# datasciencetoolkit/NextGP.jl

Measured on AMD Instinct MI355X. Metric: gibbs_iterations_per_sec, higher is better.
Workload: dtype f64; 1 GPU; single-trait Gibbs sweep, N=50000 individuals x P=600000 SNPs, marker sets BayesPR(200000) + BayesPR(200000) + BayesPR(200000), fp32 panel in HBM (BASELINE.json configs[3]: multi-breed random regression = three BayesPR marker sets of 200,000 SNPs); N=50000, P=600000, chains=1, panel_dtype=f32, accumulate_dtype=f64

## Files before the change

__graft_entry__.py:

```python
import os
import subprocess
import sys

ROOT = os.path.dirname(os.path.abspath(__file__))
PKG = os.path.join(ROOT, "nextgp.jl_amd")
CSRC = os.path.join(PKG, "csrc")
LIB = os.path.join(PKG, "libnextgp_hip.so")
HIPCC = os.environ.get("HIPCC", "/opt/rocm/bin/hipcc")
HIP_FLAGS = ["--offload-arch=gfx950", "-O3", "-std=c++17", "-ffp-contract=off", "-fPIC"]
OBJ_DIR = os.path.join(ROOT, "build", "obj")
_SWEEP_DEPS = ["ngp_sweep_inst.hip", "ngp_sweep.h", "ngp_sweep_body.inc", "ngp_sweep_multi_body.inc", "ngp_sweep_args.h", "ngp_common.h", "ngp_rng.h"]
UNITS = [("ngp_api.o", "ngp_api.hip", [], ["ngp_api.hip", "ngp_kernels.h", "ngp_state.h", "ngp_random.h", "ngp_random_tuple.h", "ngp_dense.h", "ngp_logvar.h", "ngp_bayesrc.h", "ngp_predict.h", "ngp_holdout.h", "ngp_genvar.h", "ngp_sweep_args.h", "ngp_common.h", "ngp_rng.h"]),
         ("ngp_genvar.o", "ngp_genvar_inst.hip", [], ["ngp_genvar_inst.hip", "ngp_genvar.h", "ngp_common.h"]),
         ("ngp_sweep_0.o", "ngp_sweep_inst.hip", ["-DNGP_INST_DBG=0"], _SWEEP_DEPS),
         ("ngp_sweep_1.o", "ngp_sweep_inst.hip", ["-DNGP_INST_DBG=1"], _SWEEP_DEPS),
         ("ngp_sweep_2.o", "ngp_sweep_inst.hip", ["-DNGP_INST_DBG=2"], _SWEEP_DEPS),
         ("ngp_sweep_3.o", "ngp_sweep_inst.hip", ["-DNGP_INST_DBG=3"], _SWEEP_DEPS),
         ("ngp_sweep_4.o", "ngp_sweep_inst.hip", ["-DNGP_INST_DBG=4"], _SWEEP_DEPS)]


def _stale(target, sources):
    if not os.path.exists(target):
        return True
    t = os.path.getmtime(target)
    return any(os.path.getmtime(s) > t for s in sources)


def build(force=False):
    srcs = [os.path.join(CSRC, f) for f in sorted(os.listdir(CSRC))] + [os.path.join(ROOT, "include", "nextgp_hip.h")]
    if force or _stale(LIB, srcs):
        os.makedirs(OBJ_DIR, exist_ok=True)
        procs = []
        hdr = os.path.join(ROOT, "include", "nextgp_hip.h")
# ... 57 lines not shown
```

nextgp.jl_amd/_lib.py:

```python
import ctypes as C
import os

import numpy as np

_HERE = os.path.dirname(os.path.abspath(__file__))
LIB_PATH = os.environ.get("NGP_HIP_LIB") or os.path.join(_HERE, "libnextgp_hip.so")

METHOD_BAYESPR, METHOD_BAYESB, METHOD_BAYESC, METHOD_BAYESR, METHOD_TUPLE, METHOD_BAYESLV, METHOD_BAYESRC = 0, 1, 2, 3, 4, 5, 6
LV_MAXCOV, LV_WORDS = 16, 17


def _sample_header(f, path):
    magic = f.read(8)
    if magic not in (b"NGPSMP01", b"NGPSMP02", b"NGPSMP03", b"NGPSMP04"):
        raise NextGPHipError(f"not a sample file: {path}")
    P, nvb, nsets, nfix, ncls, rec = (int(v) for v in np.frombuffer(f.read(48), dtype=np.int64))
    sets = [dict(zip(("method", "K", "col0", "ncol", "nvb", "tk"), np.frombuffer(f.read(48), dtype=np.int64).tolist())) for _ in range(nsets)]
    rq = []
    if magic in (b"NGPSMP02", b"NGPSMP03", b"NGPSMP04"):
        nr = int(np.frombuffer(f.read(8), dtype=np.int64)[0])
        rq = np.frombuffer(f.read(8 * nr), dtype=np.int64).tolist()
    lv = []
    if magic in (b"NGPSMP03", b"NGPSMP04"):
        nl = int(np.frombuffer(f.read(8), dtype=np.int64)[0])
# ... 955 lines not shown
    def set_trace_loci(self, loci, n_varBeta=0):
        loci = np.ascontiguousarray(loci, dtype=np.int64)
        self._chk(self.L.ngp_set_trace_loci(self.h, _p(loci, C.c_int64) if len(loci) else None, C.c_int64(len(loci)), C.c_int64(n_varBeta)))
        self.ntl, self.ntvb = len(loci), n_varBeta

    def get_trace_ext(self, n):
        bt = np.empty((n, max(self.ntl, 1))); vt = np.empty((n, max(self.ntvb, 1))); pt = np.empty((n, max(self.nsets, 1)))
        self._chk(self.L.ngp_get_trace_ext(self.h, _p(bt, C.c_double), _p(vt, C.c_double), _p(pt, C.c_double), C.c_int64(n)))
        return dict(beta=bt[:, :self.ntl], varBeta=vt[:, :self.ntvb], pi=pt[:, :self.nsets])

    def census(self):
        g, r, e = C.c_int64(), C.c_int64(), C.c_int32()
        self._chk(self.L.ngp_get_census(self.h, None, C.c_int64(0), C.byref(g), C.byref(r), C.byref(e)))
        tb = np.zeros(g.value, dtype=np.uint64)
        self._chk(self.L.ngp_get_census(self.h, _p(tb, C.c_uint64), C.c_int64(g.value), None, None, None))
        return dict(grid=g.value, retries=r.value, exclusive=bool(e.value), xcc=(tb >> np.uint64(32)).astype(np.int64) - 1,
                    hw_id=(tb & np.uint64(0xFFFFFFFF)).astype(np.int64))

    def warmer(self):
        a, b = C.c_int32(), C.c_int64()
        self._chk(self.L.ngp_get_warmer(self.h, C.byref(a), C.byref(b)))
        return dict(active=a.value, blocks=b.value)

    def debug_fail_census(self, iteration):
        self._chk(self.L.ngp_debug_fail_census(self.h, C.c_int64(iteration)))

    def debug_set_virtual_device(self, vdev):
        self._chk(self.L.ngp_debug_set_virtual_device(self.h, C.c_int32(vdev)))

    @staticmethod
    def allreduce_posterior(samplers):
        L = samplers[0].L
# ... 30 lines not shown
```

nextgp.jl_amd/csrc/ngp_api.hip:

```cpp
#include <hip/hip_runtime.h>
#include <cassert>

#include <dlfcn.h>

#include <algorithm>
#include <chrono>
#include <cmath>
#include <cstdio>
#include <cstdlib>
#include <condition_variable>
#include <cstddef>
#include <cstring>
#include <array>
#include <atomic>
#include <deque>
#include <map>
#include <memory>
#include <mutex>
#include <queue>
#include <string>
#include <thread>
#include <vector>

#include "../../include/nextgp_hip.h"
// ... 199 lines not shown
constexpr size_t NGP_LDS_MAX = 160 * 1024;

void choose_layout(int64_t N, int64_t max_shards, int64_t r_cap, int64_t *R, int64_t *S, bool prefer_odd = true) {
    int64_t r0 = (N + max_shards - 1) / max_shards;
    int64_t m = (r0 + 3) / 4;
    if (m < 1) m = 1;
    if (prefer_odd && (m & 1) == 0 && 4 * (m + 1) <= r_cap) m += 1;
    int64_t r = 4 * m;
    if (r > r_cap) r = r_cap;
    *R = r;
    *S = (N + r - 1) / r;
}

size_t sampler_lds(SweepKernel k) {
    const size_t base = (size_t)(3 * 4096 + 2 * NGP_RING * NGP_BLK + 6 * NGP_BLK) * sizeof(double) + 2 * NGP_BLK * sizeof(int) + 320;
    if (k == SweepKernel::lean) return base;
    if (k == SweepKernel::r || k == SweepKernel::multi_r) return base + NGP_SAMPLER_TUPLE_LDS + NGP_SAMPLER_R_LDS;
    return base + NGP_SAMPLER_TUPLE_LDS;
}

size_t streamer_lds(const SweepPlan &p, int K) {
    const int R = (int)p.R;
    if (K > 1) return p.streamer == 3 ? ngp_rows_multi_lds_bytes(R, K, true) : (p.streamer == 2 ? ngp_rows_multi_lds_bytes(R, K) : ngp_multi_lds_bytes(R, K));
    if (p.streamer >= 2) {
        const size_t nq = (p.streamer == 3) ? (size_t)R / 16 : (size_t)R / 4, hq = std::min<size_t>(NGP_ROWS_HMAX, (nq + 1) / 2);
        return (2 * nq + hq) * NGP_QS + (size_t)p.V * ((R + 7) & ~7) * 8 + 2 * NGP_ROWS_NW * NGP_BLK * 8 + 2 * NGP_DLS * 8 + 16 * 8 + 64 + 1024;
    }
    return 2 * (size_t)(R / 4) * NGP_QS + (size_t)R * 16 + 4096 + 2 * 512 + 128 + 3072 + (size_t)R * 64;
}

size_t sweep_lds(const SweepPlan &p, SweepKernel k, int K = 1) {
// ... 12 lines not shown
        assert(!diag && (K == 1 || p.V == 1));
        return K > 1 ? SweepKernel::multi_rc : (p.V > 1 ? SweepKernel::tall_rc : SweepKernel::rc);
    }
    if (K > 1) {
        if (rset && sweep_lds(p, SweepKernel::multi_r, K) <= NGP_LDS_MAX) return SweepKernel::multi_r;
        return tup ? SweepKernel::multi_tup : SweepKernel::multi;
    }
    if (p.V > 1) return SweepKernel::tall;
    if (diag) return SweepKernel::diag;
    if (rset && sweep_lds(p, SweepKernel::r) <= NGP_LDS_MAX) return SweepKernel::r;
    if (tup || rset) return SweepKernel::tup;
    return SweepKernel::lean;
}

const void *sweep_kernel(SweepKernel k) {
    for (auto unit : {sweep_kernel_0, sweep_kernel_1, sweep_kernel_2, sweep_kernel_3, sweep_kernel_4})
        if (const void *f = unit(k)) return f;
    return nullptr;
}

void launch_sweep_kernel(SweepKernel k, int64_t grid, size_t lds, hipStream_t stream, void *args) {
    void *a[] = {args};
    (void)hipLaunchKernel(sweep_kernel(k), dim3((unsigned)grid), dim3(NGP_WG), a, lds, stream);
}

int plan_sweep(int64_t N, int cu_count, const PlanRequest &q, SweepPlan *out, const char **msg) {
    SweepPlan p;
    p.mode = q.mode;
    int64_t max_shards = cu_count - 1 - (cu_count + NGP_GRP - 1) / NGP_GRP;
    if (q.max_shards_req > 0) max_shards = std::min<int64_t>(max_shards, q.max_shards_req);
    if (q.storage == 1) {
// ... 349 lines not shown
    if ((rc = c.d_ycorr.alloc(h, (size_t)L))) return rc;
    if (!h->h_rw.empty()) {
        std::vector<double> rs((size_t)L, 0.0);
        for (int64_t i = 0; i < N; i++) rs[(size_t)i] = std::sqrt(h->h_rw[(size_t)i]);
        if ((rc = c.d_rs.alloc(h, (size_t)L))) return rc;
        HCHK(hipMemcpy(c.d_rs, rs.data(), rs.size() * sizeof(double), hipMemcpyHostToDevice));
    }
    if ((rc = c.d_part.alloc(h, (size_t)plan.S * NGP_BLK))) return rc;
    if ((rc = c.d_dlt.alloc(h, NGP_BLK))) return rc;
    if ((rc = c.d_sets.alloc(h, 16))) return rc;
    if ((rc = c.d_scal.alloc(h, 1))) return rc;
    HCHK(hipMemsetAsync(c.d_setof, 0xFF, pp, h->stream));
    HCHK(hipMemsetAsync(c.d_delta, 1, pp, h->stream));
    if (req.storage == 0) HCHK(hipFuncSetAttribute((const void *)k_step, hipFuncAttributeMaxDynamicSharedMemorySize, (int)lds_step));
    if (plan.mode == 1) {
        for (SweepKernel k : {SweepKernel::lean, SweepKernel::diag, SweepKernel::tup, SweepKernel::r, SweepKernel::rc, SweepKernel::tall, SweepKernel::tall_rc}) {
            const size_t lds = sweep_lds(plan, k);
            if (lds <= NGP_LDS_MAX) HCHK(hipFuncSetAttribute(sweep_kernel(k), hipFuncAttributeMaxDynamicSharedMemorySize, (int)lds));
        }
        int wg_per_cu = 0;
        const SweepKernel occ = plan.V > 1 ? SweepKernel::tall : SweepKernel::lean;
        HCHK(hipOccupancyMaxActiveBlocksPerMultiprocessor(&wg_per_cu, sweep_kernel(occ), NGP_WG, sweep_lds(plan, SweepKernel::tup)));
        const int64_t grid = sweep_grid(plan);
        if (wg_per_cu < 1 || grid > (int64_t)wg_per_cu * h->cu_count)
            return fail(h, NGP_ERR_STATE, "persistent sweep: grid of " + std::to_string(grid) + " workgroups cannot be co-resident (" +
                                              std::to_string(wg_per_cu) + " per CU x " + std::to_string(h->cu_count) + " CUs); use ngp_configure(mode 0)");
        if ((rc = c.d_cdlt.alloc(h, (size_t)NGP_RING * NGP_BLK))) return rc;
        if ((rc = c.d_cdltg.alloc(h, (size_t)NGP_RING * NGP_BLK * 2))) return rc;
        c.census_off = (size_t)NGP_RING * NGP_FX_COPIES * NGP_BLK * 2 + 32;
        c.ccnt_words = c.census_off + 32 + 2 * (size_t)320;
        if ((rc = c.d_ccnt.alloc(h, c.ccnt_words))) return rc;
// ... 219 lines not shown
        if ((rc = h->mm.d_tseg_len.alloc(h, h->h_tseg_len.size()))) return rc;
        if ((rc = h->mm.d_tseg_set.alloc(h, h->h_tseg_set.size()))) return rc;
        if ((rc = h->mm.d_tsegpart.alloc(h, h->h_tseg_l0.size() * NGP_TPAIRS))) return rc;
        HCHK(hipMemcpy(h->mm.d_tregs, h->h_tregs.data(), h->h_tregs.size() * sizeof(DTReg), hipMemcpyHostToDevice));
        HCHK(hipMemcpy(h->mm.d_tseg_l0, h->h_tseg_l0.data(), h->h_tseg_l0.size() * sizeof(long long), hipMemcpyHostToDevice));
        HCHK(hipMemcpy(h->mm.d_tseg_len, h->h_tseg_len.data(), h->h_tseg_len.size() * sizeof(int32_t), hipMemcpyHostToDevice));
        HCHK(hipMemcpy(h->mm.d_tseg_set, h->h_tseg_set.data(), h->h_tseg_set.size() * sizeof(int32_t), hipMemcpyHostToDevice));
    }
    h->tables_dirty = false;
    return NGP_OK;
}

bool is_kept(const ngp_handle *h, int64_t it) {
    if (it < h->burnIn + h->thin || it > h->chainLength) return false;
    return ((it - h->burnIn) % h->thin) == 0;
}

void fill_sweep_args(ngp_handle *h, int64_t tb0, int64_t tb1, SweepArgs &A) {
    const int R = (int)h->plan.R, S = (int)h->plan.S;
    A.tiles = h->pm->tiles; A.ycorr = h->cm.d_ycorr; A.gramx = h->pm->gramx;
    const bool tf = wants_tinv(h) && h->cm.tinv_blocks == h->NBLK;
    A.tinv = (tf && h->cm.lin_any) ? h->cm.d_tinv : nullptr;
    A.blin = (tf && h->cm.lin_any) ? h->cm.d_blin : nullptr;
    A.lin_all = (tf && h->cm.lin_any) ? h->cm.lin_all : 0;
    A.V = h->plan.V; A.D = h->plan.D; A.R = R; A.S = S; A.NG = h->plan.NG; A.near = h->plan.near; A.fine_ok = 0; A.t0 = (int)tb0; A.t1 = (int)tb1;
    A.beta = h->cm.d_beta; A.delta = h->cm.d_delta; A.c = h->cm.d_c; A.w = h->cm.d_w; A.q = h->cm.d_q; A.mpm = h->pm->mpm; A.chi = h->cm.d_chi;
    A.setof = h->cm.d_setof; A.vbidx = h->cm.d_vbidx; A.sets = h->cm.d_sets; A.varBeta = h->mm.d_varBeta;
    A.rcls = h->mm.d_rcls; A.rhs0 = h->cm.d_rhs0; A.scal = h->cm.d_scal; A.Ppad = h->Ppad;
    A.tup = h->ntuple ? h->mm.d_tup : nullptr; A.tupc = h->mm.d_tupc; A.tupg = h->mm.d_tupg;
    A.acc = (unsigned long long *)h->cm.d_ccnt.get(); A.dlt = h->cm.d_cdlt; A.dltg = h->cm.d_cdltg;
    h->launch_seq = (h->launch_seq % 4095u) + 1u;
    A.nonce = h->launch_seq;
    A.flag_dlt = h->cm.d_ccnt + (size_t)NGP_RING * NGP_FX_COPIES * NGP_BLK * 2; A.abort_w = h->cm.d_abort; A.xcc_w = h->cm.d_abort + 16;
    A.census = (h->dbg_mode == 0) ? h->cm.d_ccnt + h->cm.census_off : nullptr;
    A.census_tbl = h->cm.d_census_tbl; A.iter_tag = (unsigned)(h->iter + 1);
    A.census_fail = (h->dbg_census_fail_iter > 0 && !h->exclusive) ? (unsigned)h->dbg_census_fail_iter : 0u;
    A.dbg = h->hm.d_dbg;
    A.fine_ok = (streamer_lds(h->plan, 1) + 8192 <= sweep_lds(h->plan, SweepKernel::diag)) ? 1 : 0;
    const bool warmer_tall = h->plan.R >= NGP_WARMER_MIN_R || (h->knob & NGP_KNOB_WARMER_ANY_R);
    const bool warmer_idle = h->plan.NG > 0 && h->plan.NG % 8 == 0 && h->plan.near + h->plan.NG >= h->plan.D;
    const bool warmer = h->dbg_mode == 0 && h->plan.streamer == 2 && h->plan.V == 1 && !(h->knob & NGP_KNOB_NO_WARMER) &&
                        warmer_tall && warmer_idle;
    A.variant = h->plan.streamer; A.knob = (h->knob & ~NGP_KNOB_WARMER) | (warmer ? NGP_KNOB_WARMER : 0);
    A.mean = h->pm->mean; A.N = h->N;
    A.dbg_mode = h->dbg_mode;
}

void launch_sweep(ngp_handle *h, int64_t tb0, int64_t tb1, hipEvent_t *evs) {
    const int R = (int)h->plan.R, S = (int)h->plan.S;
    if (h->plan.mode == 1) {
        SweepArgs A;
        fill_sweep_args(h, tb0, tb1, A);
        const SweepKernel k = pick_kernel(h->plan, 1, h->hm.d_dbg || h->dbg_mode, h->ntuple > 0, h->nclass_total > 0, !h->mm.rc.empty());
        h->last_grid = sweep_grid(h->plan);
        if (evs) (void)hipEventRecord(evs[0], h->stream);
        launch_sweep_kernel(k, h->last_grid, sweep_lds(h->plan, k), h->stream, &A);
        if (evs) (void)hipEventRecord(evs[1], h->stream);
        h->sweep_launches += 1;
        return;
    }
    int e = 0;
    for (int64_t t = tb0; t <= tb1; t++) {
        const int do_upd = t > tb0, do_gemv = t < tb1;
        if (evs && do_gemv) (void)hipEventRecord(evs[e++], h->stream);
        hipLaunchKernelGGL(k_step, dim3((unsigned)S), dim3(256), h->lds_step, h->stream, h->pm->tiles, h->cm.d_ycorr, h->cm.d_dlt, h->cm.d_part, R,
                           S, (int)t, do_upd, do_gemv);
        if (evs && do_gemv) (void)hipEventRecord(evs[e++], h->stream);
        if (do_gemv)
// ... 4273 lines not shown
```

nextgp.jl_amd/csrc/ngp_sweep.h:

```cpp
#pragma once
#include <cstddef>
#include <type_traits>
#include "ngp_sweep_args.h"

#ifndef NGP_ROWS_DPP
#define NGP_ROWS_DPP 1
#endif

#pragma clang fp contract(off)

namespace ngp {


#define NGP_DBG_FOLD                                                     \
    unsigned long long *const dbg = DBG ? A.dbg : nullptr;               \
    const int dbg_mode = DBG ? A.dbg_mode : 0;                           \
    (void)dbg; (void)dbg_mode;
#define NGP_DBG_LOCALS                                                   \
    unsigned long long *const dbg = A.dbg;                               \
    const int dbg_mode = A.dbg_mode;                                     \
    (void)dbg; (void)dbg_mode;
#define NGP_DBG_ROWS NGP_DBG_FOLD

__device__ inline unsigned ld_u32(const unsigned *p) { return __hip_atomic_load(p, __ATOMIC_RELAXED, __HIP_MEMORY_SCOPE_AGENT); }
// ... 503 lines not shown
#define NGP_VMC8(b) NGP_VMC(b) NGP_VMC(b + 1) NGP_VMC(b + 2) NGP_VMC(b + 3) NGP_VMC(b + 4) NGP_VMC(b + 5) NGP_VMC(b + 6) NGP_VMC(b + 7)
    switch (n) {
        NGP_VMC(1) NGP_VMC(2) NGP_VMC(3) NGP_VMC(4) NGP_VMC(5) NGP_VMC(6) NGP_VMC(7) NGP_VMC(8) NGP_VMC(9) NGP_VMC(10) NGP_VMC(11)
        NGP_VMC(12) NGP_VMC(13) NGP_VMC(14) NGP_VMC(15) NGP_VMC(16) NGP_VMC(17) NGP_VMC(18) NGP_VMC(19) NGP_VMC(20) NGP_VMC(21)
        NGP_VMC(22) NGP_VMC(23) NGP_VMC(24) NGP_VMC(25) NGP_VMC(26) NGP_VMC(27) NGP_VMC(28) NGP_VMC(29) NGP_VMC(30) NGP_VMC(31)
        NGP_VMC(32) NGP_VMC(33) NGP_VMC(34) NGP_VMC(35) NGP_VMC(36) NGP_VMC(37) NGP_VMC(38) NGP_VMC(39) NGP_VMC(40) NGP_VMC(41)
        NGP_VMC(42) NGP_VMC(43) NGP_VMC(44) NGP_VMC(45) NGP_VMC(46) NGP_VMC(47) NGP_VMC(48) NGP_VMC(49) NGP_VMC(50) NGP_VMC(51)
        NGP_VMC(52) NGP_VMC(53) NGP_VMC(54) NGP_VMC(55) NGP_VMC(56) NGP_VMC(57) NGP_VMC(58) NGP_VMC(59) NGP_VMC(60) NGP_VMC(61)
        NGP_VMC(62) NGP_VMC(63)
        default: asm volatile("s_waitcnt vmcnt(0)" ::: "memory"); break;
    }
#undef NGP_VMC8
#undef NGP_VMC
}

template <bool DBG, int DT, int ST>
__device__ __attribute__((always_inline)) inline void role_streamer_rows(const SweepArgs &A, const int s, char *smem) {
    NGP_DBG_ROWS
    constexpr bool U8 = (ST != 0);
    constexpr int NT = U8 ? ST : 1;
    const int R = A.R, S = A.S, tid = threadIdx.x;
    const int wv = __builtin_amdgcn_readfirstlane(tid >> 6), lane = tid & 63;
    const int NQ = U8 ? (R >> 4) : (R >> 2);
    const int H = min(NGP_ROWS_HMAX, (NQ + 1) >> 1);
    const int RQ = 2 * NQ + H;
    char *ring = smem;
    double *ys = (double *)(smem + (size_t)RQ * NGP_QS);
    double *red = ys + ((R + 7) & ~7);
    double *dl = red + 2 * NGP_ROWS_NW * NGP_BLK;
    double *rsy = dl + 2 * NGP_DLS;
    int *sflag = (int *)(rsy + 16);
    char *scratch = (char *)(rsy + 16) + 64;
    unsigned long long *fine = (unsigned long long *)(scratch + 1024);
    const bool fine_on = DBG && dbg && s == (DBG ? fine_shard(A) : 1) && A.fine_ok == 1;
#define NGP_FINE(k)                                                                                              \
    do {                                                                                                         \
        if (fine_on && (unsigned)(u - 800) < 16u && lane == 0) fine[(((u - 800) * 8 + wv) << 3) + (k)] = wall_clock64(); \
    } while (0)
    const size_t tile_bytes = (size_t)NQ * 1024;
    double *yg = A.ycorr + (size_t)s * R;
    const int g = s / NGP_GRP;
    const int nb = A.t1 - A.t0;
    for (int i = tid; i < R; i += NGP_WG) ys[i] = yg[i];
    int *gcnt0 = (int *)(rsy + 7), *gcnt1 = (int *)(rsy + 15);
    const bool early = U8 ? ((A.knob & 256) != 0) : ((A.knob & 256) == 0);
    if (tid == 0) { *sflag = 1; *gcnt0 = 0; *gcnt1 = 0; }
    int base = 0;
    auto wrap = [&](int p) __attribute__((always_inline)) { return p >= RQ ? p - RQ : p; };
    if (wv == NGP_ROWS_NW) {
        const unsigned ring0 = (unsigned)(size_t)(__attribute__((address_space(3))) const char *)ring;
        const unsigned scratch0 = (unsigned)(size_t)(__attribute__((address_space(3))) const char *)scratch;
        const unsigned voff = (unsigned)lane * 16u;
        const bool no_dma = DBG && dbg_mode == 4;
        const int pace = A.knob & 7;
        auto dma_quads = [&](int tile, int q0, int q1, int tbase) __attribute__((always_inline)) {
            if (no_dma || q0 >= q1) return 0;
            const char *g = (const char *)A.tiles + ((size_t)(A.t0 + tile) * S + s) * tile_bytes + (size_t)q0 * 1024;
            int p = wrap(tbase + q0);
            int q = q0;
            for (; q + 4 <= q1; q += 4) {
                if (p + 4 <= RQ) {
                    dma16_s4(ring0 + (unsigned)p * NGP_QS, g, voff);
// ... 16 lines not shown
            }
            for (; q < q1; ++q) {
                dma16_s(ring0 + (unsigned)p * NGP_QS, g, voff);
                g += 1024;
                if (++p == RQ) p = 0;
            }
            return q1 - q0;
        };
        const unsigned my_xcc = xcc_id() + 1u;
        const int nslice = max(1, S / 8);
        const int slice = (s / 8) % nslice;
        const size_t gram_bytes = warm_bytes(A, min(DT, A.near + 1)), w_thi = warm_t_hi(A), w_shift = warm_shift(A);
        const size_t slice_bytes = ((gram_bytes / nslice + 1023) / 1024) * 1024;
        bool same_xcd = false, xcc_known = false;
        __builtin_amdgcn_s_setprio(3);
        if (nb > 0) dma_quads(0, 0, NQ, 0);
        if (nb > 1) dma_quads(1, 0, H, NQ);
        drain_vm();
        wg_barrier();
        for (int u = 0; u < nb + DT; ++u) {
            NGP_FINE(0);
            const int base1 = wrap(base + NQ), base2 = wrap(base1 + NQ);
            if (!xcc_known && (u & 7) == 0) {
                if constexpr (U8) {
                    const unsigned x = sld_u32(A.xcc_w);
                    xcc_known = (x != 0u);
                    same_xcd = (x == my_xcc);
                } else {
                    unsigned x, wx = 0u;
                    if (A.knob & NGP_KNOB_WARMER) sld_u32x2_glc(A.xcc_w, warmer_words(A), x, wx);
                    else x = sld_u32(A.xcc_w);
                    xcc_known = (x != 0u) && (x != my_xcc || !(A.knob & NGP_KNOB_WARMER) || wx != 0u);
                    same_xcd = (x == my_xcc) && (wx != x) && !(A.knob & NGP_KNOB_NO_WARM);
                }
            }
            if (same_xcd && u + 1 < nb && !no_dma) {
                const char *gb = (const char *)(A.gramx + (size_t)(A.t0 + u + 1) * DT * NGP_BLK * NGP_BLK) - w_shift;
                const char *tb = (const char *)(A.tinv + (size_t)(A.t0 + u + 1) * NGP_BLK * NGP_BLK);
                const size_t lo = (size_t)slice * slice_bytes, hi = min((size_t)(slice + 1) * slice_bytes, gram_bytes);
                for (size_t off = lo; off + 1024 <= hi; off += 1024) dma16_warm(scratch0, (off < w_thi ? tb : gb) + off, voff);
            }
            if (u + 1 < nb) dma_quads(u + 1, H, NQ, base1);
            int n2 = 0;
            if (u + 2 < nb) n2 = dma_quads(u + 2, 0, H, base2);
            NGP_FINE(1);
            wait_vmcnt_le(n2);
            NGP_FINE(2);
            wg_barrier();
            if (!*sflag) return;
            base = base1;
        }
        drain_vm();
    } else {
        const int c = lane & 7, ql = lane >> 3;
        const int nqw = (NQ - wv + NGP_ROWS_NW - 1) / NGP_ROWS_NW;
        int tslot[NT], trow[NT];
        bool thas[NT];
#pragma unroll
        for (int i = 0; i < NT; i++) {
            if constexpr (U8) {
                const int tau = ql + 8 * i;
                thas[i] = (tau >> 2) < nqw;
                tslot[i] = thas[i] ? wv + NGP_ROWS_NW * (tau >> 2) : wv;
                trow[i] = 16 * tslot[i] + 4 * (tau & 3);
            } else {
                const int qt = wv + NGP_ROWS_NW * ql;
                thas[i] = qt < NQ;
                tslot[i] = thas[i] ? qt : wv;
                trow[i] = 4 * qt;
            }
// ... 7 lines not shown
            for (int jj = 0; jj < 8; jj++) {
                if constexpr (U8) {
#pragma unroll
                    for (int i = 0; i < NT; i++) keep8[d][i][jj] = 0u;
                } else {
                    keep[d][jj] = make_float4(0.f, 0.f, 0.f, 0.f);
                }
            }
        unsigned long long pg0 = 0, pg1 = 0;
        double pm = 0.0;
        int pm_blk = -1;
        double mpub = 0.0;
        if (U8 && wv == NGP_ROWS_PUBW && nb > 0) mpub = A.mean[(size_t)A.t0 * NGP_BLK + lane];
        const double fxs = A.scal->fx_scale;
        auto try_signal = [&](bool) __attribute__((always_inline)) {};
        auto publish = [&](const int u) __attribute__((always_inline)) {
            const int slot = u % NGP_RING;
            const double *rp = red + (u & 1) * NGP_ROWS_NW * NGP_BLK + lane;
            double p = ((rp[0] + rp[NGP_BLK]) + (rp[2 * NGP_BLK] + rp[3 * NGP_BLK])) + ((rp[4 * NGP_BLK] + rp[5 * NGP_BLK]) + rp[6 * NGP_BLK]);
            if constexpr (U8) {
                const double *sp = rsy + (u & 1) * 8;
                const double sy = ((sp[0] + sp[1]) + (sp[2] + sp[3])) + ((sp[4] + sp[5]) + sp[6]);
                const double ms = mpub * sy;
                p = p - ms;
            }
            if (U8 && u + 1 < nb) mpub = A.mean[(size_t)(A.t0 + u + 1) * NGP_BLK + lane];
            acc_add(A.acc, A.abort_w, slot, s, lane, p, fxs);
            if (DBG && dbg && s == 0 && lane == 0) dbg[NGP_DBG_STREAM + 2 * (size_t)u] = wall_clock64();
        };
        wg_barrier();
// ... 77 lines not shown
                            }
                            const double q4 = (y0 + y1) + (y2 + y3);
                            vsum = (i == 0) ? q4 : vsum + q4;
                        }
                    }
                    if (u < nb) {
                        vsum = vsum + dpp_f64(vsum, 4);
                        const double r0 = readlane_d(vsum, 0), r1 = readlane_d(vsum, 16), r2 = readlane_d(vsum, 32), r3 = readlane_d(vsum, 48);
                        if (lane == 0) rsy[(u & 1) * 8 + wv] = (r0 + r1) + (r2 + r3);
                    }
                }
                NGP_FINE(1);
                try_signal(false);
                if (u < nb) {
                    double acc = 0.0;
                    for (int k = 0; k < nqw; k++) {
                        const int q = wv + NGP_ROWS_NW * k;
                        if constexpr (U8) {
                            const uint4 x = *(const uint4 *)(ring + (size_t)wrap(base + q) * NGP_QS + (size_t)lane * 16);
                            const double *yq = ys + 16 * q;
                            const unsigned xw[4] = {x.x, x.y, x.z, x.w};
#pragma unroll
                            for (int e4 = 0; e4 < 4; e4++) {
                                const unsigned w = xw[e4];
                                const double y0 = yq[4 * e4], y1 = yq[4 * e4 + 1], y2 = yq[4 * e4 + 2], y3 = yq[4 * e4 + 3];
                                acc = __builtin_fma((double)(float)(w & 0xffu), y0, acc);
                                acc = __builtin_fma((double)(float)((w >> 8) & 0xffu), y1, acc);
                                acc = __builtin_fma((double)(float)((w >> 16) & 0xffu), y2, acc);
                                acc = __builtin_fma((double)(float)(w >> 24), y3, acc);
                            }
                        } else {
// ... 1 lines not shown
#if NGP_ROWS_DPP
                            const double xd[4] = {(double)x.x, (double)x.y, (double)x.z, (double)x.w};
                            double yv[1] = {ys[4 * q + (lane & 3)]}, ac[1] = {acc};
                            fmac4_bcast<1>(ac, yv, xd);
                            acc = ac[0];
#else
                            const double *yq = ys + 4 * q;
                            const double y0 = yq[0], y1 = yq[1], y2 = yq[2], y3 = yq[3];
                            acc = __builtin_fma((double)x.x, y0, acc);
                            acc = __builtin_fma((double)x.y, y1, acc);
                            acc = __builtin_fma((double)x.z, y2, acc);
                            acc = __builtin_fma((double)x.w, y3, acc);
#endif
                        }
                    }
                    red[((u & 1) * NGP_ROWS_NW + wv) * NGP_BLK + lane] = acc;
                    if (early) {
                        asm volatile("" ::: "memory");
                        if (lane == 0) __hip_atomic_fetch_add((lds_int_t *)((u & 1) ? gcnt1 : gcnt0), 1, __ATOMIC_RELAXED, __HIP_MEMORY_SCOPE_WORKGROUP);
                    }
                    NGP_FINE(2);
                    try_signal(false);
                    if constexpr (U8) {
#pragma unroll
                        for (int i = 0; i < NT; i++) {
                            const char *tq = ring + (size_t)wrap(base + tslot[i]) * NGP_QS + c * 128 + (trow[i] & 15);
#pragma unroll
                            for (int jj = 0; jj < 8; jj++) keep8[d][i][jj] = *(const unsigned *)(tq + jj * 16);
                        }
                    } else {
                        const char *tq = ring + (size_t)wrap(base + tslot[0]) * NGP_QS + c * 128;
#pragma unroll
                        for (int jj = 0; jj < 8; jj++) keep[d][jj] = *(const float4 *)(tq + jj * 16);
                    }
                }
                NGP_FINE(3);
                if (early && wv == NGP_ROWS_PUBW && u < nb && !(DBG && dbg_mode == 1)) {
// ... 42 lines not shown
                NGP_FINE(5);
                if (!early && wv == NGP_ROWS_PUBW && u < nb && !(DBG && dbg_mode == 1)) publish(u);
                base = wrap(base + NQ);
                NGP_FINE(6);
            }
        }
        try_signal(true);
    }
    if (fine_on && nb > 816) {
        __syncthreads();
        for (int i = tid; i < 1024; i += NGP_WG) dbg[NGP_DBG_ALL + 8192 + i] = fine[i];
    }
#undef NGP_FINE
    __syncthreads();
    for (int i = tid; i < R; i += NGP_WG) yg[i] = ys[i];
}

template <int DT, int V>
__device__ __attribute__((always_inline)) inline void role_streamer_rows_tall(const SweepArgs &A, const int s, char *smem) {
    const int R = A.R, S = A.S, tid = threadIdx.x;
    const int wv = __builtin_amdgcn_readfirstlane(tid >> 6), lane = tid & 63;
    const int NQ = R >> 2;
    const int H = min(NGP_ROWS_HMAX, (NQ + 1) >> 1);
    const int RQ = 2 * NQ + H;
    const int RP = (R + 7) & ~7;
    char *ring = smem;
    double *ys = (double *)(smem + (size_t)RQ * NGP_QS);
    double *red = ys + V * RP;
    double *dl = red + 2 * NGP_ROWS_NW * NGP_BLK;
    double *rsy = dl + 2 * NGP_DLS;
// ... 1056 lines not shown
        }
        if (verdict != 1u) {
            st_u32(A.abort_w + 1, A.iter_tag);
            st_u32(A.abort_w, NGP_ABORT_CENSUS);
        }
        *cflag = (verdict == 1u) ? 1 : 0;
    }
    __syncthreads();
    const int cok = *cflag;
    __syncthreads();
    return cok != 0;
}

template <bool DBG>
__global__ __launch_bounds__(NGP_WG) __attribute__((amdgpu_waves_per_eu(2, 2))) void k_sweep(SweepArgs A) {
    constexpr bool TUP = DBG;
    constexpr int RCLSV = DBG ? 1 : 0;
#include "ngp_sweep_body.inc"
}
#if defined(NGP_INST_DBG) && NGP_INST_DBG == 2
__global__ __launch_bounds__(NGP_WG) __attribute__((amdgpu_waves_per_eu(2, 2))) void k_sweep_tup(SweepArgs A) {
    constexpr bool DBG = false, TUP = true;
    constexpr int RCLSV = 1;
#include "ngp_sweep_body.inc"
}
#endif
#if defined(NGP_INST_DBG) && NGP_INST_DBG == 3
__global__ __launch_bounds__(NGP_WG) __attribute__((amdgpu_waves_per_eu(2, 2))) void k_sweep_r(SweepArgs A) {
    constexpr bool DBG = false, TUP = true;
    constexpr int RCLSV = 2;
#include "ngp_sweep_body.inc"
}
#endif
#if defined(NGP_INST_DBG) && NGP_INST_DBG == 4
__global__ __launch_bounds__(NGP_WG) __attribute__((amdgpu_waves_per_eu(2, 2))) void k_sweep_rc(SweepArgs A) {
    constexpr bool DBG = false, TUP = true;
    constexpr int RCLSV = 3;
#include "ngp_sweep_body.inc"
}
__global__ __launch_bounds__(NGP_WG) __attribute__((amdgpu_waves_per_eu(2, 2))) void k_sweep_tall_rc(SweepArgs A) {
    extern __shared__ __attribute__((aligned(16))) char smem[];
    const int b = blockIdx.x;
    if (ld_u32(A.abort_w) != 0u) return;
    if (!sweep_census(A, b, smem)) return;
    if (b == 0)
        role_sampler<false, true, true, 3>(A, smem);
    else if (b <= A.NG)
        role_reducer<false>(A, b - 1, smem);
    else if (A.V == 2)
        role_streamer_rows_tall<3, 2>(A, b - 1 - A.NG, smem);
    else
// ... 672 lines not shown
```

nextgp.jl_amd/csrc/ngp_sweep_args.h:

```cpp
#pragma once
#include "ngp_common.h"

#define NGP_RING 16
#define NGP_MAX_LAG 12
#define NGP_SPIN_LIMIT (1u << 21)
#define NGP_WG 512
#define NGP_DBG_WAVES (1u << 19)
#define NGP_DBG_RED (3u << 18)
#define NGP_DBG_W5 (5u << 17)
#define NGP_DBG_ALL (7u << 17)
#define NGP_DBG_RELOOK (NGP_DBG_ALL - 3)
#define NGP_SPARSE_MAX 16
#ifndef NGP_LAZY_LAG
#define NGP_LAZY_LAG 7
#endif
#define NGP_QS 1040
#define NGP_SAMPLER_TUPLE_LDS (2 * 9 * 64 * 8 + 64)
#define NGP_SAMPLER_R_LDS (2 * 17 * 64 * 8 + 2 * 128 * 4 + 64 + 2 * 16 * 64 * 8)
#define NGP_ABORT_CENSUS 9u
#define NGP_CENSUS_TICKS 2000000ull
#define NGP_DBG_STREAM (1u << 20)
#define NGP_KNOB_NO_WARM 2048
#define NGP_KNOB_WARMER 4096
#define NGP_KNOB_NO_WARMER 8192
#define NGP_KNOB_WARMER_ANY_R 16384
#define NGP_WARMER_MIN_R 160

namespace ngp {

struct SweepArgs {
    const float *tiles;
    double *ycorr;
    const double *gramx;
    const double *tinv;
    const unsigned *blin;
    int lin_all;
    int knob;
    int variant;
    int V;
    int D, R, S, NG, near, fine_ok, t0, t1;
// ... 20 lines not shown
    unsigned *abort_w;
    unsigned *census;
    unsigned long long *census_tbl;
    unsigned iter_tag;
    unsigned census_fail;
    unsigned *xcc_w;
    unsigned long long *dbg;
    int dbg_mode;
};

#define NGP_ROWS_MAX_R 224
#define NGP_ROWS_NW 7
#ifndef NGP_ROWS_HMAX
#define NGP_ROWS_HMAX 32
#endif
#define NGP_ROWS_PUBW 2
#define NGP_ROWS_POLLW 6
#define NGP_DLS 72

__host__ __device__ inline int ngp_u8_tasks(int R) {
    const int nuw = ((R >> 4) + NGP_ROWS_NW - 1) / NGP_ROWS_NW;
    const int nt = (4 * nuw + 7) / 8;
    return nt <= 1 ? 1 : (nt == 2 ? 2 : 4);
}
#define NGP_U8_MAX_R 896

#ifndef NGP_MAXC
#define NGP_MAXC 8
#endif
#ifndef NGP_PAIR_FROM
// ... 9 lines not shown
    unsigned long long *acc;
    const double *dlt;
    const unsigned *flag_dlt;
};
__host__ __device__ inline size_t ngp_multi_chain_doubles(int R) { return (size_t)R + 512 + 128 + (size_t)8 * R; }
__host__ __device__ inline size_t ngp_multi_lds_bytes(int R, int K) {
    return (size_t)2 * (R >> 2) * NGP_QS + (size_t)K * ngp_multi_chain_doubles(R) * 8 + 64 + 3072;
}

__host__ __device__ inline size_t ngp_rows_multi_chain_doubles(int R) { return (size_t)((R + 7) & ~7) + 2 * NGP_ROWS_NW * NGP_BLK + 2 * NGP_DLS + 16; }
__host__ __device__ inline size_t ngp_rows_multi_lds_bytes(int R, int K, bool u8 = false) {
    const size_t nq = (size_t)R / (u8 ? 16 : 4), hq = nq + 1 < 2 * (size_t)NGP_ROWS_HMAX ? (nq + 1) / 2 : (size_t)NGP_ROWS_HMAX;
    return (2 * nq + hq) * NGP_QS + (size_t)K * ngp_rows_multi_chain_doubles(R) * 8 + 64 + 64 + 1024;
}

enum class SweepKernel { lean, diag, tup, r, tall, multi, multi_tup, multi_r, rc, tall_rc, multi_rc };
const void *sweep_kernel_0(SweepKernel k);
const void *sweep_kernel_1(SweepKernel k);
const void *sweep_kernel_2(SweepKernel k);
const void *sweep_kernel_3(SweepKernel k);
const void *sweep_kernel_4(SweepKernel k);

}
```

nextgp.jl_amd/csrc/ngp_sweep_body.inc:

```
    extern __shared__ __attribute__((aligned(16))) char smem[];
    NGP_DBG_LOCALS
    const int b = blockIdx.x;
    if (ld_u32(A.abort_w) != 0u) return;
    if (!sweep_census(A, b, smem)) return;
    if (dbg_mode == 1 && b <= A.NG) return;
    if ((dbg_mode == 2 && b != 0) || ((dbg_mode == 3 || dbg_mode == 4) && b == 0)) return;
    if (b == 0)
        role_sampler<DBG, false, TUP, RCLSV>(A, smem);
    else if (b <= A.NG) {
        if (b == A.NG && (A.knob & NGP_KNOB_WARMER)) role_warmer<DBG>(A, smem);
        else role_reducer<DBG>(A, b - 1, smem);
    } else {
        const int s = b - 1 - A.NG;
        if (A.variant == 2) {
            switch (A.D) {
                case 3: role_streamer_rows<DBG, 3, 0>(A, s, smem); break;
                case 4: role_streamer_rows<DBG, 4, 0>(A, s, smem); break;
                case 5: role_streamer_rows<DBG, 5, 0>(A, s, smem); break;
                default: role_streamer_rows<DBG, 6, 0>(A, s, smem); break;
            }
            return;
        }
        if (A.variant == 3) {
            const int nt = ngp_u8_tasks(A.R);
            if (nt == 1) {
                switch (A.D) {
                    case 3: role_streamer_rows<DBG, 3, 1>(A, s, smem); break;
                    case 4: role_streamer_rows<DBG, 4, 1>(A, s, smem); break;
                    case 6: role_streamer_rows<DBG, 6, 1>(A, s, smem); break;
                    case 8: role_streamer_rows<DBG, 8, 1>(A, s, smem); break;
                    default: role_streamer_rows<DBG, 12, 1>(A, s, smem); break;
                }
            } else if (nt == 2) {
                if (A.D == 4) role_streamer_rows<DBG, 4, 2>(A, s, smem);
// ... 36 lines not shown
```

nextgp.jl_amd/csrc/ngp_sweep_inst.hip:

```cpp
#include <hip/hip_runtime.h>

#include "ngp_sweep.h"

#ifndef NGP_INST_DBG
#error "compile with -DNGP_INST_DBG=0, 1, 2, 3 or 4"
#endif

#define NGP_CAT_(a, b) a##b
#define NGP_CAT(a, b) NGP_CAT_(a, b)

namespace ngp {

const void *NGP_CAT(sweep_kernel_, NGP_INST_DBG)(SweepKernel k) {
    switch (k) {
#if NGP_INST_DBG == 0
    case SweepKernel::lean: return (const void *)k_sweep<false>;
    case SweepKernel::multi: return (const void *)k_sweep_multi;
#elif NGP_INST_DBG == 1
    case SweepKernel::diag: return (const void *)k_sweep<true>;
    case SweepKernel::tall: return (const void *)k_sweep_tall;
#elif NGP_INST_DBG == 2
    case SweepKernel::tup: return (const void *)k_sweep_tup;
    case SweepKernel::multi_tup: return (const void *)k_sweep_multi_tup;
#elif NGP_INST_DBG == 3
    case SweepKernel::r: return (const void *)k_sweep_r;
    case SweepKernel::multi_r: return (const void *)k_sweep_multi_r;
#elif NGP_INST_DBG == 4
    case SweepKernel::rc: return (const void *)k_sweep_rc;
    case SweepKernel::tall_rc: return (const void *)k_sweep_tall_rc;
    case SweepKernel::multi_rc: return (const void *)k_sweep_multi_rc;
#endif
    default: return nullptr;
    }
}

}
```

Baseline: 47.44 it/s.

## Load last row-quads per wave directly from global in streamer rows kernel

Adds a lean_dq sweep kernel variant in which each compute wave loads its final quad(s) of the fp32 tile straight from global memory into registers, prefetched one tile ahead. It then writes them into the LDS ring itself and accumulates them, so the DMA wave moves fewer quads per tile. The intent is to shorten the DMA wave's critical path in the streamer-rows pipeline. In exchange the compute waves issue extra global loads and LDS stores, and a new kernel instantiation is added. It is gated on streamer==2, V==1, fp32 storage and R>=160, and a census counter records how many quads were loaded directly.

```diff
diff --git a/__graft_entry__.py b/__graft_entry__.py
--- a/__graft_entry__.py
+++ b/__graft_entry__.py
@@ -16,7 +16,8 @@
          ("ngp_sweep_1.o", "ngp_sweep_inst.hip", ["-DNGP_INST_DBG=1"], _SWEEP_DEPS),
          ("ngp_sweep_2.o", "ngp_sweep_inst.hip", ["-DNGP_INST_DBG=2"], _SWEEP_DEPS),
          ("ngp_sweep_3.o", "ngp_sweep_inst.hip", ["-DNGP_INST_DBG=3"], _SWEEP_DEPS),
-         ("ngp_sweep_4.o", "ngp_sweep_inst.hip", ["-DNGP_INST_DBG=4"], _SWEEP_DEPS)]
+         ("ngp_sweep_4.o", "ngp_sweep_inst.hip", ["-DNGP_INST_DBG=4"], _SWEEP_DEPS),
+         ("ngp_sweep_5.o", "ngp_sweep_inst.hip", ["-DNGP_INST_DBG=5"], _SWEEP_DEPS)]
 
 
 def _stale(target, sources):
diff --git a/nextgp.jl_amd/_lib.py b/nextgp.jl_amd/_lib.py
--- a/nextgp.jl_amd/_lib.py
+++ b/nextgp.jl_amd/_lib.py
@@ -993,8 +993,8 @@
         self._chk(self.L.ngp_get_census(self.h, None, C.c_int64(0), C.byref(g), C.byref(r), C.byref(e)))
         tb = np.zeros(g.value, dtype=np.uint64)
         self._chk(self.L.ngp_get_census(self.h, _p(tb, C.c_uint64), C.c_int64(g.value), None, None, None))
-        return dict(grid=g.value, retries=r.value, exclusive=bool(e.value), xcc=(tb >> np.uint64(32)).astype(np.int64) - 1,
-                    hw_id=(tb & np.uint64(0xFFFFFFFF)).astype(np.int64))
+        return dict(grid=g.value, retries=r.value, exclusive=bool(e.value), xcc=((tb >> np.uint64(32)) & np.uint64(0xFF)).astype(np.int64) - 1,
+                    hw_id=(tb & np.uint64(0xFFFFFFFF)).astype(np.int64), direct=(tb >> np.uint64(40)).astype(np.int64))
 
     def warmer(self):
         a, b = C.c_int32(), C.c_int64()
diff --git a/nextgp.jl_amd/csrc/ngp_api.hip b/nextgp.jl_amd/csrc/ngp_api.hip
--- a/nextgp.jl_amd/csrc/ngp_api.hip
+++ b/nextgp.jl_amd/csrc/ngp_api.hip
@@ -237,7 +237,7 @@
 
 size_t sampler_lds(SweepKernel k) {
     const size_t base = (size_t)(3 * 4096 + 2 * NGP_RING * NGP_BLK + 6 * NGP_BLK) * sizeof(double) + 2 * NGP_BLK * sizeof(int) + 320;
-    if (k == SweepKernel::lean) return base;
+    if (k == SweepKernel::lean || k == SweepKernel::lean_dq) return base;
     if (k == SweepKernel::r || k == SweepKernel::multi_r) return base + NGP_SAMPLER_TUPLE_LDS + NGP_SAMPLER_R_LDS;
     return base + NGP_SAMPLER_TUPLE_LDS;
 }
@@ -280,7 +280,7 @@
 }
 
 const void *sweep_kernel(SweepKernel k) {
-    for (auto unit : {sweep_kernel_0, sweep_kernel_1, sweep_kernel_2, sweep_kernel_3, sweep_kernel_4})
+    for (auto unit : {sweep_kernel_0, sweep_kernel_1, sweep_kernel_2, sweep_kernel_3, sweep_kernel_4, sweep_kernel_5})
         if (const void *f = unit(k)) return f;
     return nullptr;
 }
@@ -660,7 +660,7 @@
     HCHK(hipMemsetAsync(c.d_delta, 1, pp, h->stream));
     if (req.storage == 0) HCHK(hipFuncSetAttribute((const void *)k_step, hipFuncAttributeMaxDynamicSharedMemorySize, (int)lds_step));
     if (plan.mode == 1) {
-        for (SweepKernel k : {SweepKernel::lean, SweepKernel::diag, SweepKernel::tup, SweepKernel::r, SweepKernel::rc, SweepKernel::tall, SweepKernel::tall_rc}) {
+        for (SweepKernel k : {SweepKernel::lean, SweepKernel::lean_dq, SweepKernel::diag, SweepKernel::tup, SweepKernel::r, SweepKernel::rc, SweepKernel::tall, SweepKernel::tall_rc}) {
             const size_t lds = sweep_lds(plan, k);
             if (lds <= NGP_LDS_MAX) HCHK(hipFuncSetAttribute(sweep_kernel(k), hipFuncAttributeMaxDynamicSharedMemorySize, (int)lds));
         }
@@ -910,6 +910,12 @@
 bool is_kept(const ngp_handle *h, int64_t it) {
     if (it < h->burnIn + h->thin || it > h->chainLength) return false;
     return ((it - h->burnIn) % h->thin) == 0;
+}
+
+static bool sweep_direct_quads(const ngp_handle *h) {
+    const int nq = (int)h->plan.R / 4, hq = std::min<int>(NGP_ROWS_HMAX, (nq + 1) / 2);
+    return h->plan.mode == 1 && h->plan.streamer == 2 && h->plan.V == 1 && h->req.storage == 0 && !(h->knob & NGP_KNOB_NO_DIRECT) &&
+           nq - NGP_ROWS_NW * NGP_ROWS_DIRECT >= hq && (h->plan.R >= NGP_DIRECT_MIN_R || (h->knob & NGP_KNOB_DIRECT_ANY_R));
 }
 
 void fill_sweep_args(ngp_handle *h, int64_t tb0, int64_t tb1, SweepArgs &A) {
@@ -937,7 +943,7 @@
     const bool warmer_idle = h->plan.NG > 0 && h->plan.NG % 8 == 0 && h->plan.near + h->plan.NG >= h->plan.D;
     const bool warmer = h->dbg_mode == 0 && h->plan.streamer == 2 && h->plan.V == 1 && !(h->knob & NGP_KNOB_NO_WARMER) &&
                         warmer_tall && warmer_idle;
-    A.variant = h->plan.streamer; A.knob = (h->knob & ~NGP_KNOB_WARMER) | (warmer ? NGP_KNOB_WARMER : 0);
+    A.variant = h->plan.streamer; A.knob = (h->knob & ~(NGP_KNOB_WARMER | NGP_KNOB_DIRECT)) | (warmer ? NGP_KNOB_WARMER : 0) | (sweep_direct_quads(h) ? NGP_KNOB_DIRECT : 0);
     A.mean = h->pm->mean; A.N = h->N;
     A.dbg_mode = h->dbg_mode;
 }
@@ -947,7 +953,9 @@
     if (h->plan.mode == 1) {
         SweepArgs A;
         fill_sweep_args(h, tb0, tb1, A);
-        const SweepKernel k = pick_kernel(h->plan, 1, h->hm.d_dbg || h->dbg_mode, h->ntuple > 0, h->nclass_total > 0, !h->mm.rc.empty());
+        SweepKernel k = pick_kernel(h->plan, 1, h->hm.d_dbg || h->dbg_mode, h->ntuple > 0, h->nclass_total > 0, !h->mm.rc.empty());
+        if (k == SweepKernel::lean && (A.knob & NGP_KNOB_DIRECT)) k = SweepKernel::lean_dq;
+        else if (k != SweepKernel::diag) A.knob &= ~NGP_KNOB_DIRECT;
         h->last_grid = sweep_grid(h->plan);
         if (evs) (void)hipEventRecord(evs[0], h->stream);
         launch_sweep_kernel(k, h->last_grid, sweep_lds(h->plan, k), h->stream, &A);
diff --git a/nextgp.jl_amd/csrc/ngp_sweep.h b/nextgp.jl_amd/csrc/ngp_sweep.h
--- a/nextgp.jl_amd/csrc/ngp_sweep.h
+++ b/nextgp.jl_amd/csrc/ngp_sweep.h
@@ -541,7 +541,7 @@
 #undef NGP_VMC
 }
 
-template <bool DBG, int DT, int ST>
+template <bool DBG, int DT, int ST, bool DQ = false>
 __device__ __attribute__((always_inline)) inline void role_streamer_rows(const SweepArgs &A, const int s, char *smem) {
     NGP_DBG_ROWS
     constexpr bool U8 = (ST != 0);
@@ -551,6 +551,10 @@
     const int NQ = U8 ? (R >> 4) : (R >> 2);
     const int H = min(NGP_ROWS_HMAX, (NQ + 1) >> 1);
     const int RQ = 2 * NQ + H;
+    constexpr int KD = NGP_ROWS_DIRECT;
+    static_assert(!DQ || !U8, "direct quads: fp32 tiles only");
+    const bool direct = DQ ? (A.knob & NGP_KNOB_DIRECT) != 0 : false;
+    const int NQD = DQ ? (direct ? NQ - NGP_ROWS_NW * KD : NQ) : NQ;
     char *ring = smem;
     double *ys = (double *)(smem + (size_t)RQ * NGP_QS);
     double *red = ys + ((R + 7) & ~7);
@@ -573,6 +577,7 @@
     const bool early = U8 ? ((A.knob & 256) != 0) : ((A.knob & 256) == 0);
     if (tid == 0) { *sflag = 1; *gcnt0 = 0; *gcnt1 = 0; }
     int base = 0;
+    int ndirect = 0;
     auto wrap = [&](int p) __attribute__((always_inline)) { return p >= RQ ? p - RQ : p; };
     if (wv == NGP_ROWS_NW) {
         const unsigned ring0 = (unsigned)(size_t)(__attribute__((address_space(3))) const char *)ring;
@@ -619,7 +624,7 @@
         const size_t slice_bytes = ((gram_bytes / nslice + 1023) / 1024) * 1024;
         bool same_xcd = false, xcc_known = false;
         __builtin_amdgcn_s_setprio(3);
-        if (nb > 0) dma_quads(0, 0, NQ, 0);
+        if (nb > 0) dma_quads(0, 0, NQD, 0);
         if (nb > 1) dma_quads(1, 0, H, NQ);
         drain_vm();
         wg_barrier();
@@ -645,7 +650,7 @@
                 const size_t lo = (size_t)slice * slice_bytes, hi = min((size_t)(slice + 1) * slice_bytes, gram_bytes);
                 for (size_t off = lo; off + 1024 <= hi; off += 1024) dma16_warm(scratch0, (off < w_thi ? tb : gb) + off, voff);
             }
-            if (u + 1 < nb) dma_quads(u + 1, H, NQ, base1);
+            if (u + 1 < nb) dma_quads(u + 1, H, NQD, base1);
             int n2 = 0;
             if (u + 2 < nb) n2 = dma_quads(u + 2, 0, H, base2);
             NGP_FINE(1);
@@ -659,6 +664,7 @@
     } else {
         const int c = lane & 7, ql = lane >> 3;
         const int nqw = (NQ - wv + NGP_ROWS_NW - 1) / NGP_ROWS_NW;
+        const int nqg = DQ ? (direct ? nqw - KD : nqw) : nqw;
         int tslot[NT], trow[NT];
         bool thas[NT];
 #pragma unroll
@@ -696,6 +702,16 @@
         if (U8 && wv == NGP_ROWS_PUBW && nb > 0) mpub = A.mean[(size_t)A.t0 * NGP_BLK + lane];
         const double fxs = A.scal->fx_scale;
         auto try_signal = [&](bool) __attribute__((always_inline)) {};
+        float4 dq0 = make_float4(0.f, 0.f, 0.f, 0.f), dq1 = dq0;
+        const bool direct_ld = direct && !(DBG && dbg_mode == 4);
+        auto direct_request = [&](const int tile) __attribute__((always_inline)) {
+            const char *g = (const char *)A.tiles + ((size_t)(A.t0 + tile) * S + s) * tile_bytes + (size_t)(wv + NGP_ROWS_NW * nqg) * 1024 + (size_t)lane * 16;
+            dq0 = *(const float4 *)g;
+            if constexpr (KD > 1) dq1 = *(const float4 *)(g + NGP_ROWS_NW * 1024);
+        };
+        if constexpr (DQ) {
+            if (direct_ld && nb > 0) direct_request(0);
+        }
         auto publish = [&](const int u) __attribute__((always_inline)) {
             const int slot = u % NGP_RING;
             const double *rp = red + (u & 1) * NGP_ROWS_NW * NGP_BLK + lane;
@@ -803,7 +819,7 @@
                 try_signal(false);
                 if (u < nb) {
                     double acc = 0.0;
-                    for (int k = 0; k < nqw; k++) {
+                    for (int k = 0; k < nqg; k++) {
                         const int q = wv + NGP_ROWS_NW * k;
                         if constexpr (U8) {
                             const uint4 x = *(const uint4 *)(ring + (size_t)wrap(base + q) * NGP_QS + (size_t)lane * 16);
@@ -835,6 +851,30 @@
 #endif
                         }
                     }
+                    if constexpr (DQ) {
+                        if (direct) {
+                            ndirect += KD;
+#pragma unroll
+                            for (int i = 0; i < KD; i++) {
+                                const int q = wv + NGP_ROWS_NW * (nqg + i);
+                                const float4 x = i ? dq1 : dq0;
+                                *(float4 *)(ring + (size_t)wrap(base + q) * NGP_QS + (size_t)lane * 16) = x;
+#if NGP_ROWS_DPP
+                                const double xd[4] = {(double)x.x, (double)x.y, (double)x.z, (double)x.w};
+                                double yv[1] = {ys[4 * q + (lane & 3)]}, ac[1] = {acc};
+                                fmac4_bcast<1>(ac, yv, xd);
+                                acc = ac[0];
+#else
+                                const double *yq = ys + 4 * q;
+                                const double y0 = yq[0], y1 = yq[1], y2 = yq[2], y3 = yq[3];
+                                acc = __builtin_fma((double)x.x, y0, acc);
+                                acc = __builtin_fma((double)x.y, y1, acc);
+                                acc = __builtin_fma((double)x.z, y2, acc);
+                                acc = __builtin_fma((double)x.w, y3, acc);
+#endif
+                            }
+                        }
+                    }
                     red[((u & 1) * NGP_ROWS_NW + wv) * NGP_BLK + lane] = acc;
                     if (early) {
                         asm volatile("" ::: "memory");
@@ -842,6 +882,10 @@
                     }
                     NGP_FINE(2);
                     try_signal(false);
+                    if constexpr (DQ) {
+                        asm volatile("" ::: "memory");
+                        if (direct_ld && u + 1 < nb) direct_request(u + 1);
+                    }
                     if constexpr (U8) {
 #pragma unroll
                         for (int i = 0; i < NT; i++) {
@@ -914,6 +958,9 @@
 #undef NGP_FINE
     __syncthreads();
     for (int i = tid; i < R; i += NGP_WG) yg[i] = ys[i];
+    if constexpr (DQ) {
+        if (direct && A.census && tid == 0) A.census_tbl[1 + A.NG + s] += (unsigned long long)ndirect << 40;
+    }
 }
 
 template <int DT, int V>
@@ -2000,27 +2047,34 @@
 
 template <bool DBG>
 __global__ __launch_bounds__(NGP_WG) __attribute__((amdgpu_waves_per_eu(2, 2))) void k_sweep(SweepArgs A) {
-    constexpr bool TUP = DBG;
+    constexpr bool TUP = DBG, DQV = DBG;
     constexpr int RCLSV = DBG ? 1 : 0;
 #include "ngp_sweep_body.inc"
 }
+#if defined(NGP_INST_DBG) && NGP_INST_DBG == 5
+__global__ __launch_bounds__(NGP_WG) __attribute__((amdgpu_waves_per_eu(2, 2))) void k_sweep_dq(SweepArgs A) {
+    constexpr bool DBG = false, TUP = false, DQV = true;
+    constexpr int RCLSV = 0;
+#include "ngp_sweep_body.inc"
+}
+#endif
 #if defined(NGP_INST_DBG) && NGP_INST_DBG == 2
 __global__ __launch_bounds__(NGP_WG) __attribute__((amdgpu_waves_per_eu(2, 2))) void k_sweep_tup(SweepArgs A) {
-    constexpr bool DBG = false, TUP = true;
+    constexpr bool DBG = false, TUP = true, DQV = false;
     constexpr int RCLSV = 1;
 #include "ngp_sweep_body.inc"
 }
 #endif
 #if defined(NGP_INST_DBG) && NGP_INST_DBG == 3
 __global__ __launch_bounds__(NGP_WG) __attribute__((amdgpu_waves_per_eu(2, 2))) void k_sweep_r(SweepArgs A) {
-    constexpr bool DBG = false, TUP = true;
+    constexpr bool DBG = false, TUP = true, DQV = false;
     constexpr int RCLSV = 2;
 #include "ngp_sweep_body.inc"
 }
 #endif
 #if defined(NGP_INST_DBG) && NGP_INST_DBG == 4
 __global__ __launch_bounds__(NGP_WG) __attribute__((amdgpu_waves_per_eu(2, 2))) void k_sweep_rc(SweepArgs A) {
-    constexpr bool DBG = false, TUP = true;
+    constexpr bool DBG = false, TUP = true, DQV = false;
     constexpr int RCLSV = 3;
 #include "ngp_sweep_body.inc"
 }
diff --git a/nextgp.jl_amd/csrc/ngp_sweep_args.h b/nextgp.jl_amd/csrc/ngp_sweep_args.h
--- a/nextgp.jl_amd/csrc/ngp_sweep_args.h
+++ b/nextgp.jl_amd/csrc/ngp_sweep_args.h
@@ -24,6 +24,10 @@
 #define NGP_KNOB_WARMER 4096
 #define NGP_KNOB_NO_WARMER 8192
 #define NGP_KNOB_WARMER_ANY_R 16384
+#define NGP_KNOB_NO_DIRECT 32768
+#define NGP_KNOB_DIRECT_ANY_R (1 << 28)
+#define NGP_KNOB_DIRECT (1 << 29)
+#define NGP_DIRECT_MIN_R 160
 #define NGP_WARMER_MIN_R 160
 
 namespace ngp {
@@ -74,6 +78,9 @@
 #ifndef NGP_ROWS_HMAX
 #define NGP_ROWS_HMAX 32
 #endif
+#ifndef NGP_ROWS_DIRECT
+#define NGP_ROWS_DIRECT 1
+#endif
 #define NGP_ROWS_PUBW 2
 #define NGP_ROWS_POLLW 6
 #define NGP_DLS 72
@@ -113,11 +120,12 @@
     return (2 * nq + hq) * NGP_QS + (size_t)K * ngp_rows_multi_chain_doubles(R) * 8 + 64 + 64 + 1024;
 }
 
-enum class SweepKernel { lean, diag, tup, r, tall, multi, multi_tup, multi_r, rc, tall_rc, multi_rc };
+enum class SweepKernel { lean, diag, tup, r, tall, multi, multi_tup, multi_r, rc, tall_rc, multi_rc, lean_dq };
 const void *sweep_kernel_0(SweepKernel k);
 const void *sweep_kernel_1(SweepKernel k);
 const void *sweep_kernel_2(SweepKernel k);
 const void *sweep_kernel_3(SweepKernel k);
 const void *sweep_kernel_4(SweepKernel k);
+const void *sweep_kernel_5(SweepKernel k);
 
 }
diff --git a/nextgp.jl_amd/csrc/ngp_sweep_body.inc b/nextgp.jl_amd/csrc/ngp_sweep_body.inc
--- a/nextgp.jl_amd/csrc/ngp_sweep_body.inc
+++ b/nextgp.jl_amd/csrc/ngp_sweep_body.inc
@@ -14,10 +14,10 @@
         const int s = b - 1 - A.NG;
         if (A.variant == 2) {
             switch (A.D) {
-                case 3: role_streamer_rows<DBG, 3, 0>(A, s, smem); break;
-                case 4: role_streamer_rows<DBG, 4, 0>(A, s, smem); break;
-                case 5: role_streamer_rows<DBG, 5, 0>(A, s, smem); break;
-                default: role_streamer_rows<DBG, 6, 0>(A, s, smem); break;
+                case 3: role_streamer_rows<DBG, 3, 0, DQV>(A, s, smem); break;
+                case 4: role_streamer_rows<DBG, 4, 0, DQV>(A, s, smem); break;
+                case 5: role_streamer_rows<DBG, 5, 0, DQV>(A, s, smem); break;
+                default: role_streamer_rows<DBG, 6, 0, DQV>(A, s, smem); break;
             }
             return;
         }
diff --git a/nextgp.jl_amd/csrc/ngp_sweep_inst.hip b/nextgp.jl_amd/csrc/ngp_sweep_inst.hip
--- a/nextgp.jl_amd/csrc/ngp_sweep_inst.hip
+++ b/nextgp.jl_amd/csrc/ngp_sweep_inst.hip
@@ -3,7 +3,7 @@
 #include "ngp_sweep.h"
 
 #ifndef NGP_INST_DBG
-#error "compile with -DNGP_INST_DBG=0, 1, 2, 3 or 4"
+#error "compile with -DNGP_INST_DBG=0, 1, 2, 3, 4 or 5"
 #endif
 
 #define NGP_CAT_(a, b) a##b
@@ -29,6 +29,8 @@
     case SweepKernel::rc: return (const void *)k_sweep_rc;
     case SweepKernel::tall_rc: return (const void *)k_sweep_tall_rc;
     case SweepKernel::multi_rc: return (const void *)k_sweep_multi_rc;
+#elif NGP_INST_DBG == 5
+    case SweepKernel::lean_dq: return (const void *)k_sweep_dq;
 #endif
     default: return nullptr;
     }
```

New measurement: 48.28 it/s (median of 6 runs). 1.02x the previous value.
